# ZhengyiLuo/SMPLSim

Hardware: AMD Instinct MI355X
Metric: env-steps/sec (whole node), 4096-env SMPL rollout at 1/2/4/8 MI355X (higher is better)
Workload: dtype f32

## Files before the change

smplsim_amd/csrc/ss_api.h:

```cpp
#pragma once
#include <cassert>
#include <cstdlib>
#include <new>
#include <string>

#include "ss_imfused.h"
#include "ss_mjcf.h"
#include "ss_tables.h"

namespace ss {
inline std::string &last_error() { static thread_local std::string e; return e; }
inline std::string *&error_slot() { static thread_local std::string *p = nullptr; return p; }
struct HandleScope {
  template <class H> explicit HandleScope(const H *handle) { error_slot() = handle ? &handle->err : nullptr; }
  ~HandleScope() { error_slot() = nullptr; }
};
}

struct ss_model {
  ss::HostModel hm;
  int device = 0;
  uint32_t *d_shared = nullptr;
  ss::real *d_bodyc = nullptr, *d_candc = nullptr;
  int32_t *d_candb = nullptr;
// ... 28 lines not shown
  const float *fall_actions = nullptr;
  void *d_im = nullptr;
  ss_imitation_io im_io{};
};

template <class BE>
struct ss_api {
  static int fail(int code, const std::string &msg) {
    ss::last_error() = msg;
    if (ss::error_slot()) *ss::error_slot() = msg;
    return code;
  }

  static int model_create(const ss_model_desc *d, int device, ss_model **out) {
    if (!d || !out) return fail(SS_ERR_INVALID, "null argument");
    return model_create_shapes(d, 1, device, out);
  }
  template <class T> static bool up(T *&dst, const std::vector<T> &v) {
    const size_t bytes = v.size() * sizeof(T);
    dst = static_cast<T *>(BE::alloc(bytes ? bytes : 4));
    if (dst && bytes && !BE::upload(dst, v.data(), bytes)) { BE::free_(dst); dst = nullptr; }
    return dst != nullptr;
  }
  static int model_create_shapes(const ss_model_desc *d, int num_shapes, int device, ss_model **out) {
    if (!d || !out || num_shapes < 1) return fail(SS_ERR_INVALID, "null argument or num_shapes < 1");
    ss_model *m = new (std::nothrow) ss_model();
    if (!m) return fail(SS_ERR_NOMEM, "out of host memory");
    ss::HostModel &hm = m->hm;
    const std::string refusal = ss::build_host_model(d, num_shapes, getenv("SS_NO_ALIAS_LAYOUT") != nullptr, hm);
    if (!refusal.empty()) { delete m; return fail(SS_ERR_INVALID, refusal); }
    if (num_shapes > 1 && 12 * hm.h_sc.nb > hm.h_sc.l_Wst - hm.h_sc.l_IA) { delete m; return fail(SS_ERR_LDS, "no room for the per-env body offsets"); }
    m->num_shapes = num_shapes; m->device = device;
    if (!BE::set_device(device)) { delete m; return fail(SS_ERR_HIP, "cannot select device"); }
    if (!(up(m->d_shared, hm.shared) && up(m->d_bodyc, hm.bodyc) && up(m->d_candc, hm.candc) && up(m->d_candb, hm.candb) && up(m->d_pairs, hm.pairs) && up(m->d_geomc, hm.geomc))) {
      model_destroy(m);
      return fail(SS_ERR_HIP, "device table upload failed");
    }
    *out = m;
    return SS_OK;
  }
  static void model_destroy(ss_model *m) {
    if (!m) return;
    BE::free_(m->d_shared); BE::free_(m->d_bodyc); BE::free_(m->d_candc); BE::free_(m->d_candb); BE::free_(m->d_pairs); BE::free_(m->d_geomc);
    delete m;
  }
  static int batch_create(const ss_model *m, const ss_env_cfg *cfg, const ss_state *st, ss_batch **out) {
    if (!m || !cfg || !st || !out) return fail(SS_ERR_INVALID, "null argument");
    if (st->num_envs < 1) return fail(SS_ERR_INVALID, "num_envs must be positive");
    if (!st->qpos || !st->qvel || !st->qpos_prev || !st->qvel_prev || !st->qacc_warm || !st->body_vel || !st->touch ||
        !st->cur_t || !st->task || !st->nwarn || !st->solver_iters)
      return fail(SS_ERR_INVALID, "every ss_state buffer must be provided");
    if (cfg->control_mode < SS_CTRL_UHC_PD || cfg->control_mode > SS_CTRL_DEFAULT) return fail(SS_ERR_INVALID, "unknown control_mode");
    if (cfg->control_mode == SS_CTRL_SIMPLE_PID && (!st->pid_integral || !st->pid_last_error || !st->pid_started))
      return fail(SS_ERR_INVALID, "control_mode simple_pid needs the pid_* state buffers");
    if (cfg->self_obs_v != 1 && cfg->self_obs_v != 2) return fail(SS_ERR_INVALID, "self_obs_v must be 1 or 2");
    if (cfg->control_freq_inv < 1) return fail(SS_ERR_INVALID, "control_freq_inv must be >= 1");
    if (m->num_shapes > 1 && !st->shape_id) return fail(SS_ERR_INVALID, "a model with several shapes needs ss_state.shape_id");
    if (m->num_shapes == 1 && st->shape_id) return fail(SS_ERR_INVALID, "ss_state.shape_id given for a single-shape model");
    if (cfg->self_collision && !m->d_pairs) return fail(SS_ERR_INVALID, "model has no pair table");
    if (cfg->self_collision && !m->hm.self_collision_unavailable.empty()) return fail(SS_ERR_INVALID, m->hm.self_collision_unavailable.c_str());
    if (cfg->task == SS_TASK_REACH && (cfg->reach_body < 0 || cfg->reach_body >= m->hm.h.nb)) return fail(SS_ERR_INVALID, "reach_body out of range");
    const ss::Hdr &h = m->hm.h;
    if (ss::kernel_variant(h) < 0) return fail(SS_ERR_INVALID, "model too large for the compiled kernel variants");
    ss_batch *b = new (std::nothrow) ss_batch();
    if (!b) return fail(SS_ERR_NOMEM, "out of host memory");
    b->m = m; b->cfg = *cfg; b->st = *st;
    if (b->cfg.newton_iters <= 0) b->cfg.newton_iters = 100;
    b->cfg.solver_tolerance = (float)((cfg->solver_tolerance > 0.f ? (double)cfg->solver_tolerance : 1e-8) * m->hm.meaninertia * (h.nv > 1 ? h.nv : 1));
    b->obs_size = ss::obs_size(h, *cfg);
    size_t shared_b = (size_t)((h.shared_words + 3) & ~3) * 4;
    const size_t env_b = (size_t)(cfg->self_collision ? m->hm.sc.env_floats : h.env_floats) * sizeof(ss::real);
    int cap = BE::lds_capacity();
    const size_t pool_b = cfg->self_collision ? (size_t)ss::ss_pool_floats(m->hm.sc) * sizeof(ss::real) : 0;
    int e = (int)((cap - (long)shared_b - (long)pool_b) / (long)env_b);
    if (e < 1) { batch_destroy(b); return fail(SS_ERR_LDS, "model does not fit in LDS"); }
    { const int mw = BE::max_waves(ss::kernel_variant(h), cfg->self_collision); if (e > mw) e = mw; }
    { const char *cap = getenv("SS_ENVS_PER_WG"); if (cap && atoi(cap) > 0 && atoi(cap) < e) e = atoi(cap); }
    b->envs_per_wg = e;
    b->lds_bytes = shared_b + (size_t)e * env_b + pool_b;
#ifdef SS_PROFILE
    b->d_prof = (unsigned long long *)BE::alloc(64 * sizeof(unsigned long long));
    if (b->d_prof) { unsigned long long z[64] = {0}; BE::upload(b->d_prof, z, sizeof z); }
#endif
    if (!BE::set_device(m->device)) { batch_destroy(b); return fail(SS_ERR_HIP, "cannot select device"); }
    b->d_counter = (int32_t *)BE::alloc(2 * sizeof(int32_t));
    const int32_t zeros[2] = {0, 0};
    if (!b->d_counter || !BE::upload(b->d_counter, zeros, sizeof zeros)) { batch_destroy(b); return fail(SS_ERR_NOMEM, "device allocation failed"); }
    *out = b;
    return SS_OK;
  }
  static ss::KArgs base_args(const ss_batch *b, int mode) {
    ss::KArgs k{};
    const ss_model *m = b->m;
    k.h = b->cfg.self_collision ? m->hm.h_sc : m->hm.h; k.cfg = b->cfg; k.st = b->st;
    k.shared_g = m->d_shared; k.bodyc = m->d_bodyc; k.candc = m->d_candc; k.candb = m->d_candb;
    k.illegal_mask = m->hm.illegal_mask;
    k.hc = m->hm.hc;
    k.sc = m->hm.sc; k.pairs = m->d_pairs; k.geomc = m->d_geomc; k.dbg_self = ss_batch::R(b->dbg_self);
    k.mode = mode; k.nsub = b->cfg.control_freq_inv; k.obs_size = b->obs_size;
    k.work_counter = b->d_counter + b->parity; k.work_counter_next = b->d_counter + (b->parity ^ 1);
    k.obs_stride = b->obs_size;
    k.prof = b->d_prof;
    k.order = b->order;
// ... 248 lines not shown
```

smplsim_amd/csrc/ss_env_kernel.h:

```cpp
#pragma once
#include <hip/hip_runtime.h>

#include "ss_api.h"
#include "ss_kernel.h"
#include "ss_wave_gpu.h"

#ifndef SS_MAX_THREADS
#define SS_MAX_THREADS 768
#endif
#ifndef SS_MAX_THREADS_X
#define SS_MAX_THREADS_X 448
#endif
#ifndef SS_MAX_THREADS_SC
#define SS_MAX_THREADS_SC 512
#endif

namespace ss {
typedef void (*kern_t)(const KArgs);
kern_t pick_kernel_selfcol(const KernelKey &key, const Hdr &h, const HdrC &hc);
kern_t pick_kernel_imitation(const KernelKey &key, const Hdr &h, const HdrC &hc);
kern_t pick_kernel_imitation_selfcol(const KernelKey &key, const Hdr &h, const HdrC &hc);
kern_t pick_kernel_x(const KernelKey &key, const Hdr &h, const HdrC &hc);
}

namespace {

template <int DOFP, int CANDP, int SLOTP, int NPASS, int MAXT, bool BODYOUT, bool SHAPED, class HT = ss::HdrRuntime, bool SELFCOL = false, bool IMIT = false, bool CFORCE = false>
__global__ void __launch_bounds__(MAXT) ss_env_kernel(const ss::KArgs k) {
  extern __shared__ __align__(16) uint32_t lds[];
  if (blockIdx.x == 0 && threadIdx.x == 0) *k.work_counter_next = 0;
  for (int i = threadIdx.x; i < k.h.shared_words; i += blockDim.x) lds[i] = k.shared_g[i];
  if constexpr (SELFCOL)
    if (threadIdx.x == 0 && ss::ss_pool_floats(k.sc) > 0)
      *reinterpret_cast<int *>(reinterpret_cast<float *>(lds + ((k.h.shared_words + 3) & ~3)) + (size_t)(blockDim.x >> 6) * k.sc.env_floats) = 0;
  __syncthreads();
  const int wave = __builtin_amdgcn_readfirstlane(threadIdx.x >> 6);
  const int slice = SELFCOL ? k.sc.env_floats : HT::view(k.h).env_floats;
  float *L = reinterpret_cast<float *>(lds + ((k.h.shared_words + 3) & ~3)) + (size_t)wave * slice;
  float *pool = nullptr;
  if constexpr (SELFCOL) {
    if (ss::ss_pool_floats(k.sc) > 0) {
      pool = reinterpret_cast<float *>(lds + ((k.h.shared_words + 3) & ~3)) + (size_t)(blockDim.x >> 6) * slice;
    }
  }
  WaveGpu w{(int)(threadIdx.x & 63)};
  const int total_waves = (int)(gridDim.x * (blockDim.x >> 6));
  bool first = true;
  for (;;) {
    int env = wave * (int)gridDim.x + (int)blockIdx.x;
    if (!first) {
      if (w.ln == 0) env = atomicAdd(k.work_counter, 1) + total_waves;
      env = __builtin_amdgcn_readfirstlane(env);
    }
    first = false;
    if (env >= k.st.num_envs) break;
    if (k.order) env = __builtin_amdgcn_readfirstlane(k.order[env]);
    int mode = k.mode;
    if constexpr (IMIT) {
      const ss::mo::ImFused *f = static_cast<const ss::mo::ImFused *>(k.im);
      ss::run_env<WaveGpu, DOFP, CANDP, SLOTP, NPASS, BODYOUT, SHAPED, HT, SELFCOL, IMIT, CFORCE>(&w, &k, lds, L, env, mode, pool);
      w.sync();
      if (ss::mo::fused_after_step(&w, f, k.im_rand, env)) {
        ss::run_env<WaveGpu, DOFP, CANDP, SLOTP, NPASS, BODYOUT, SHAPED, HT, SELFCOL, IMIT, CFORCE>(&w, &k, lds, L, env, ss::MODE_RESET, pool);
        w.sync();
        ss::mo::fused_after_reset(&w, f, env);
      }
      continue;
    }
    for (int rep = 0; rep < 2; rep++) {
      const bool again = ss::run_env<WaveGpu, DOFP, CANDP, SLOTP, NPASS, BODYOUT, SHAPED, HT, SELFCOL, IMIT, CFORCE>(&w, &k, lds, L, env, mode, pool);
      w.sync();
      if (!again) break;
      mode = ss::MODE_RESET;
    }
  }
// ... 8 lines not shown
```

smplsim_amd/csrc/ss_hdr.h:

```cpp
#pragma once
#include <stdint.h>

#include "../../include/smplsim_hip.h"

#ifdef SS_F64
namespace ss { typedef double real; }
#define SS_M(fn) fn
#define SS_LS_TOL_EFF 1e-13
#define SS_ROUND_REL 2.2e-15
#define SS_DG_NOISE 1.8e-15
#define SS_LS_MAXIT 60
#else
namespace ss { typedef float real; }
#define SS_M(fn) fn##f
#define SS_LS_TOL_EFF SS_LS_TOL
#define SS_ROUND_REL 2e-6f
#define SS_DG_NOISE 1e-6f
#define SS_LS_MAXIT 16
#endif

namespace ss {

constexpr int kWave = 64;
constexpr int kBodyC = 16;
constexpr int kDofC = 12;
constexpr int kCandC = 8;

struct Hdr {
  int nb, nn, nv, nq, nu, ncand, nlev, a_stride, nbox, nslot, maxlev;
  int l_Rloc, l_w2;
  unsigned long long arm_lean;
  int o_dofc, o_boff, o_chainnode, o_ndepth, l_act, o_bparent, o_sumsmall, o_sumbig, o_sumcover, n_sumsmall, n_sumbig, shared_words;
  int l_q, l_v, l_a, l_tau, l_Fb, l_Pb, l_delta, l_diag, l_S, l_Ab, l_An, l_Aown, l_IA, l_Ubuf, l_Wst,
      l_R, l_r, l_Gb, l_tmp, l_V, l_Iown, ia_stride, env_floats;
  real dt, grav, margin, mu, solimp[5], K, B;
  real qpos0_root[3];
};

struct Layout {
  int l_q, l_v, l_a, l_tau, l_Fb, l_Pb, l_delta, l_diag, l_S, l_Ab, l_An, l_Aown, l_IA, l_Ubuf, l_Wst, l_R, l_r, l_Gb, l_tmp, l_V, l_Iown,
      ia_stride, l_act, env_floats, a_stride, l_Rloc, l_w2;
};
constexpr Layout make_layout(int nb, int maxlev, bool alias_w = false) {
  const int nn = nb + 1, nv = 6 + 3 * (nb - 1);
  Layout y{};
  int o = 0;
  auto take = [&](int n) { int r = o; o += (n + 3) & ~3; return r; };
  y.l_q = take(nv + 1); y.l_v = take(nv); y.l_a = take(nv); y.l_tau = take(nv);
  y.l_Fb = take(6 * nb);
  y.l_act = alias_w ? o : take(nv - 6);
  y.l_delta = take(nv);
// ... 17 lines not shown
    y.l_Wst = y.l_Aown;
    y.l_R = o - 12 * nb; y.l_r = y.l_R + 9 * nb;
    (void)gb; (void)t6;
    y.env_floats = o;
    return y;
  }
  y.a_stride = 21;
  y.l_Aown = take(21 * nb);
  y.ia_stride = 0;
  const int gb = (6 * nb + 3) & ~3;
  const int ia_need = 48 * maxlev > gb + 6 * nn ? 48 * maxlev : gb + 6 * nn;
  y.l_IA = take(ia_need);
  y.l_Gb = y.l_IA; y.l_tmp = y.l_IA + gb;
  y.l_Ubuf = 24 * maxlev <= 8 * nn ? y.l_An : take(24 * maxlev);
  y.l_Wst = take(24 * nn);
  y.l_R = y.l_Wst; y.l_r = y.l_Wst + 9 * nb;
  y.l_Rloc = y.l_IA; y.l_w2 = y.l_Wst + 12 * nb;
  y.env_floats = o;
  return y;
}
inline void apply_layout(Hdr &g, const Layout &y) {
  g.l_q = y.l_q; g.l_v = y.l_v; g.l_a = y.l_a; g.l_tau = y.l_tau; g.l_Fb = y.l_Fb; g.l_act = y.l_act; g.l_delta = y.l_delta; g.l_Pb = y.l_Pb; g.l_V = y.l_V;
  g.l_diag = y.l_diag; g.l_S = y.l_S; g.l_Ab = y.l_Ab; g.l_Iown = y.l_Iown; g.l_An = y.l_An; g.l_Aown = y.l_Aown; g.ia_stride = y.ia_stride;
  g.l_IA = y.l_IA; g.l_Gb = y.l_Gb; g.l_tmp = y.l_tmp; g.l_Ubuf = y.l_Ubuf; g.l_Wst = y.l_Wst; g.l_R = y.l_R; g.l_r = y.l_r;
  g.a_stride = y.a_stride; g.l_Rloc = y.l_Rloc; g.l_w2 = y.l_w2;
  g.env_floats = y.env_floats;
}
constexpr bool alias_layout_fits(int nb, int maxlev, int nslot) {
  const int nn = nb + 1;
  const Layout y = make_layout(nb, maxlev, true);
  return ((6 * nb + 3) & ~3) <= 48 * maxlev && y.l_w2 + ((6 * nn + 3) & ~3) <= y.l_R && 13 * nslot <= y.l_R - y.l_An;
}

constexpr int kMaxSelf = SS_MAX_SELF_CONTACTS;
constexpr int kSelfRec = 24;
constexpr int kSelfCand = 64;
constexpr int kCandRec = 8;
constexpr int kGeomC = 16;
constexpr int kDenseMaxRows = 64;
struct HdrSC {
  int npair;
  int l_H, l_g, l_list, l_Wst2, hloc, o_sctab, l_gc, l_tab, nmax, l_cand, l_zb;
  int env_floats;
};
constexpr int kDenseTile = 16;
constexpr int dense_tile_rows(int nblock) { return (3 * nblock + 1 + kDenseTile - 1) / kDenseTile; }
constexpr int dense_floats(int np) {
  const int t = (np - 1) / kDenseTile;
  return kDenseTile * kDenseTile * (t * (t + 1) / 2) + kDenseTile * (t + 1) * (np - kDenseTile * t);
}
constexpr int kDenseExtra = 256;
constexpr HdrSC make_layout_sc(int nb, int base_floats, int l_An) {
  HdrSC y{};
  int o = base_floats;
  auto take = [&](int n) { int r = o; o += (n + 3) & ~3; return r; };
  y.nmax = nb + 1 < kDenseMaxRows ? nb + 1 : kDenseMaxRows;
  y.l_H = l_An;
  take(kDenseExtra);
  y.hloc = o - y.l_H;
  y.l_g = take(kDenseTile * dense_tile_rows(y.nmax)); y.l_list = take(64);
  const int w2 = 24 * (nb + 1) > kCandRec * kSelfCand ? 24 * (nb + 1) : kCandRec * kSelfCand;
  y.l_Wst2 = take(w2); y.l_cand = y.l_Wst2;
  y.l_gc = take(3 * nb); y.l_zb = take(3 * nb); y.l_tab = take(3 * nb);
  y.env_floats = o;
  return y;
}
constexpr int ss_pool_floats(const HdrSC &y) { return dense_floats(3 * y.nmax + 1) > y.hloc ? 4 + ((dense_floats(3 * y.nmax + 1) + 3) & ~3) : 0; }

struct HdrC {
  int nlev;
  int o_lev;
  int root;
  int pel_level;
  unsigned long long nkpack[2];
  unsigned long long cpack;
  unsigned long long chain;
  unsigned long long neg;
};

#if defined(__HIPCC__)
#define SS_HD __host__ __device__ inline __attribute__((always_inline))
#else
#define SS_HD inline __attribute__((always_inline))
#endif
SS_HD int hdr_o_arm(const Hdr &h) { return (int)(h.arm_lean & 0xffffffffull); }
SS_HD bool hdr_lean(const Hdr &h) { return (h.arm_lean >> 32) != 0ull; }
struct HdrRuntime {
  typedef const Hdr &type;
  static constexpr bool fixed = false;
  static SS_HD bool lean(const Hdr &h) { return hdr_lean(h); }
  static constexpr bool maybe_lean = true;
  static SS_HD type view(const Hdr &h) { return h; }
  typedef const HdrC &tree_type;
  static SS_HD tree_type tree(const HdrC &c) { return c; }
};
template <int NLEV, int ROOT, int PEL, unsigned long long NK0, unsigned long long CP, unsigned long long CH, unsigned long long NG>
struct TreeFixed {
  static constexpr int nlev = NLEV, root = ROOT, pel_level = PEL;
  static constexpr unsigned long long nkpack[2] = {NK0, 0ull};
  static constexpr unsigned long long cpack = CP, chain = CH, neg = NG;
  int o_lev;
};
template <int NB, int MAXLEV, bool ALIAS = false>
struct HdrFixed {
  static constexpr Layout LY = make_layout(NB, MAXLEV, ALIAS);
  static constexpr int nb = NB, nn = NB + 1, nv = 6 + 3 * (NB - 1), nq = 7 + 3 * (NB - 1), maxlev = MAXLEV;
  static constexpr int l_q = LY.l_q, l_v = LY.l_v, l_a = LY.l_a, l_tau = LY.l_tau, l_Fb = LY.l_Fb, l_Pb = LY.l_Pb, l_delta = LY.l_delta,
                       l_diag = LY.l_diag, l_S = LY.l_S, l_Ab = LY.l_Ab, l_An = LY.l_An, l_Aown = LY.l_Aown, l_IA = LY.l_IA,
                       l_Ubuf = LY.l_Ubuf, l_Wst = LY.l_Wst, l_R = LY.l_R, l_r = LY.l_r, l_Gb = LY.l_Gb, l_tmp = LY.l_tmp, l_V = LY.l_V,
                       l_Iown = LY.l_Iown, ia_stride = LY.ia_stride, l_act = LY.l_act, env_floats = LY.env_floats,
                       a_stride = LY.a_stride, l_Rloc = LY.l_Rloc, l_w2 = LY.l_w2;
  const int &nu, &ncand, &nlev, &nbox, &nslot;
  const int &o_dofc, &o_boff, &o_chainnode, &o_ndepth, &o_bparent, &o_sumsmall, &o_sumbig, &o_sumcover, &n_sumsmall, &n_sumbig,
      &shared_words;
  const real &dt, &grav, &margin, &mu;
  const real (&solimp)[5];
  const real &K, &B;
  const real (&qpos0_root)[3];
  SS_HD explicit HdrFixed(const Hdr &h)
      : nu(h.nu), ncand(h.ncand), nlev(h.nlev), nbox(h.nbox), nslot(h.nslot), o_dofc(h.o_dofc),
        o_boff(h.o_boff), o_chainnode(h.o_chainnode), o_ndepth(h.o_ndepth), o_bparent(h.o_bparent),
        o_sumsmall(h.o_sumsmall), o_sumbig(h.o_sumbig), o_sumcover(h.o_sumcover), n_sumsmall(h.n_sumsmall), n_sumbig(h.n_sumbig),
        shared_words(h.shared_words), dt(h.dt), grav(h.grav), margin(h.margin), mu(h.mu), solimp(h.solimp), K(h.K), B(h.B),
        qpos0_root(h.qpos0_root) {}
};
template <int NB, int MAXLEV, int NLEV, int ROOT, int PEL, unsigned long long NK0, unsigned long long CP, unsigned long long CH, unsigned long long NG, bool ALIAS = false, bool LEAN = ALIAS>
struct HdrFixedT {
  typedef const HdrFixed<NB, MAXLEV, ALIAS> type;
  static constexpr bool fixed = true;
  static SS_HD constexpr bool lean(const Hdr &) { return LEAN; }
  static constexpr bool maybe_lean = LEAN;
  static SS_HD HdrFixed<NB, MAXLEV, ALIAS> view(const Hdr &h) { return HdrFixed<NB, MAXLEV, ALIAS>(h); }
  typedef const TreeFixed<NLEV, ROOT, PEL, NK0, CP, CH, NG> tree_type;
  static SS_HD TreeFixed<NLEV, ROOT, PEL, NK0, CP, CH, NG> tree(const HdrC &c) { TreeFixed<NLEV, ROOT, PEL, NK0, CP, CH, NG> t; t.o_lev = c.o_lev; return t; }
  static bool matches(const Hdr &h, const HdrC &c) {
    return h.nb == NB && h.maxlev == MAXLEV && h.a_stride == (ALIAS ? 24 : 21) && hdr_lean(h) == LEAN && h.env_floats == HdrFixed<NB, MAXLEV, ALIAS>::env_floats && c.nlev == NLEV && c.root == ROOT && c.pel_level == PEL && c.nkpack[0] == NK0 && c.nkpack[1] == 0ull && c.cpack == CP && c.chain == CH && c.neg == NG;
  }
};


typedef HdrFixedT<24, 5, 6, 10, 2, 0x333431ull, 0x1253ull, 0x1cull, 0x3ull> HdrSmplFixed;
typedef HdrFixedT<52, 12, 7, 11, 3, 0xbbb3233ull, 0x9a89ull, 0x33ull, 0x7ull, true> HdrSmplxFixed;
typedef HdrFixedT<52, 12, 7, 11, 3, 0xbbb3233ull, 0x9a89ull, 0x33ull, 0x7ull, false, true> HdrSmplxFixedSC;

inline int kernel_variant(const Hdr &h) {
  const int dofp = (h.nv + 63) / 64, candp = (h.ncand + 63) / 64, slotp = (h.nslot + 63) / 64, npass = (h.maxlev + 7) / 8;
  if (dofp <= 2 && candp <= 2 && slotp <= 1 && npass <= 1) return 0;
  if (dofp <= 3 && candp <= 3 && slotp <= 2 && npass <= 2) return 1;
  return -1;
}

template <class H> constexpr int shape_stride(const H &h) { return h.nb * kBodyC + ((h.nv + 3) & ~3); }

enum { MODE_STEP = 0, MODE_SUBSTEP = 1, MODE_RESET = 2, MODE_KINEMATICS = 3, MODE_DEBUG_FORWARD = 4 };

struct KArgs {
  Hdr h;
  ss_env_cfg cfg;
  ss_state st;
  const uint32_t *shared_g;
  const real *bodyc;
  const real *candc;
  const int32_t *candb;
  uint64_t illegal_mask;
  int mode, nsub, obs_size;
  const real *actions;
  const real *task_rand;
  const real *fall_actions;
  const uint8_t *mask;
  unsigned long long *prof;
  const int32_t *order;
  int32_t *work_counter;
  real *obs, *reward;
  int fused_reset;
  real *obs2;
  const real *task_rand2;
  uint8_t *terminated, *truncated;
  real *out0, *out1, *out2;
  HdrSC sc;
  const int32_t *pairs;
  const real *geomc;
  real *dbg_self;
  int obs_stride;
  const void *im;
  const float *im_rand;
  int32_t *work_counter_next;
  real *power;
  int32_t *self_trunc;
  HdrC hc;
  real *cforce;
};

inline int env_slice_floats(const KArgs &k) { return k.cfg.self_collision ? k.sc.env_floats : k.h.env_floats; }
inline size_t launch_lds_bytes(const KArgs &k, int e) {
  return (size_t)((k.h.shared_words + 3) & ~3) * 4 + ((size_t)e * env_slice_floats(k) + (k.cfg.self_collision ? ss_pool_floats(k.sc) : 0)) * sizeof(real);
}

struct KernelKey { int variant; bool bodyout, shaped, selfcol, imit, cforce; };
inline KernelKey kernel_key(const KArgs &k) {
  KernelKey key{kernel_variant(k.h), false, k.st.shape_id != nullptr, k.cfg.self_collision != 0, k.im != nullptr, false};
  const bool wanted = (k.out0 || k.power || k.cforce) && (k.mode == MODE_STEP || k.mode == MODE_RESET);
  key.bodyout = wanted || key.shaped || key.selfcol || key.imit;
  key.cforce = k.cforce && k.mode == MODE_STEP;
  return key;
}

struct LaunchGeometry { int wgs, envs_per_wg; size_t lds_bytes; };
inline LaunchGeometry launch_geometry(int nenv, int cus, int envs_per_wg, int fixed_epw, int max_wgs, size_t lds_capacity, size_t lds_fixed, size_t lds_per_env) {
  const int per_cu = (nenv + cus - 1) / cus;
  if (fixed_epw > 0) envs_per_wg = fixed_epw;
  else if (per_cu < envs_per_wg) envs_per_wg = per_cu < 1 ? 1 : per_cu;
  LaunchGeometry g{(nenv + envs_per_wg - 1) / envs_per_wg, envs_per_wg, lds_fixed + (size_t)envs_per_wg * lds_per_env};
  const int resident = cus * (int)(lds_capacity / g.lds_bytes > 0 ? lds_capacity / g.lds_bytes : 1);
  if (g.wgs > resident) g.wgs = resident;
  if (max_wgs > 0 && g.wgs > max_wgs) g.wgs = max_wgs;
  return g;
}

}
```

smplsim_amd/csrc/ss_kernel.h:

```cpp
#pragma once
#include <math.h>
#include <stdint.h>
#include <stdlib.h>
#include <stdio.h>

#include "ss_hdr.h"
#include "ss_selfcol.h"

#if defined(__HIPCC__)
#define SS_DEV __device__ __forceinline__
#else
#define SS_DEV inline
#endif

#ifdef SS_PROFILE
#define SS_T0() unsigned long long t__ = w->clock()
#define SS_TICK(id) do { unsigned long long n__ = w->clock(); sim.prof[id] += n__ - t__; t__ = n__; } while (0)
#else
#define SS_T0() do {} while (0)
#define SS_TICK(id) do {} while (0)
#endif

#ifndef SS_LS_TOL
#define SS_LS_TOL 1e-2f
// ... 191 lines not shown
#pragma unroll
      for (int u = 1; u < 8; u++) part[u] = u < n ? part[u] : 0.f;
      out[b * NC + c] = ((part[0] + part[1]) + (part[2] + part[3])) + ((part[4] + part[5]) + (part[6] + part[7]));
    }
    if (h.n_sumbig == 0) return;
    w->sync();
    for (int idx = lane; idx < NC * h.n_sumbig; idx += 64) {
      const int o = idx / NC, c = idx - o * NC, e = ti(h.o_sumbig, o), b = e & 255, start = (e >> 8) & 4095, cnt = e >> 20;
      real acc = 0.f;
      for (int j = 0; j < cnt; j += 4) {
        real part[4];
#pragma unroll
        for (int u = 0; u < 4; u++) {
          const int t = ti(h.o_sumcover, start + (j + u < cnt ? j + u : j));
          part[u] = (t < 64 ? in : out)[(t & 63) * NC + c];
        }
#pragma unroll
        for (int u = 1; u < 4; u++) part[u] = j + u < cnt ? part[u] : 0.f;
        acc += (part[0] + part[1]) + (part[2] + part[3]);
      }
      out[b * NC + c] = acc;
    }
  }

  SS_DEV void body_accel(const real *x, real *A, real *tmp) {
    typename HT::type h = HT::view(k->h);
    for (int idx = lane; idx < 6 * h.nn; idx += 64) {
      int n = idx / 6, c = idx - 6 * n, d = 3 * n;
      tmp[idx] = S[6 * d + c] * x[d] + S[6 * d + 6 + c] * x[d + 1] + S[6 * d + 12 + c] * x[d + 2];
    }
    w->sync();
    chain_sum(tmp, A);
  }
  SS_DEV void chain_sum(const real *tmp, real *A, const real *tmp2 = nullptr, real *A2 = nullptr) {
    typename HT::type h = HT::view(k->h);
    for (int idx = lane; idx < 6 * h.nb; idx += 64) {
      int b = idx / 6, c = idx - 6 * b, n = b + 1;
      const int dn = ti(h.o_ndepth, n), row = h.o_chainnode + n * h.nlev;
      real s = 0.f, s2 = 0.f;
      for (int kk = 0; kk <= dn; kk += 4) {
        const int k1 = kk + 1 <= dn ? kk + 1 : kk, k2 = kk + 2 <= dn ? kk + 2 : kk, k3 = kk + 3 <= dn ? kk + 3 : kk;
        const int n0 = ti(row, kk), n1 = ti(row, k1), n2 = ti(row, k2), n3 = ti(row, k3);
        const real a0 = tmp[6 * n0 + c], a1 = tmp[6 * n1 + c], a2 = tmp[6 * n2 + c], a3 = tmp[6 * n3 + c];
        s += (a0 + (kk + 1 <= dn ? a1 : 0.f)) + ((kk + 2 <= dn ? a2 : 0.f) + (kk + 3 <= dn ? a3 : 0.f));
        if (tmp2) {
          const real e0 = tmp2[6 * n0 + c], e1 = tmp2[6 * n1 + c], e2 = tmp2[6 * n2 + c], e3 = tmp2[6 * n3 + c];
          s2 += (e0 + (kk + 1 <= dn ? e1 : 0.f)) + ((kk + 2 <= dn ? e2 : 0.f) + (kk + 3 <= dn ? e3 : 0.f));
        }
      }
      A[idx] = s;
      if (tmp2) A2[idx] = s2;
    }
  }


  SS_DEV void forward_kin(bool with_dyn, bool write_sensors) {
    fresh();
    typename HT::type h = HT::view(k->h);
    SS_FT0();
    real vb[6] = {0, 0, 0, 0, 0, 0}, ab[6] = {0, 0, 0, 0, 0, 0};
    real Rb[9] = {1, 0, 0, 0, 1, 0, 0, 0, 1}, rb[3] = {0, 0, 0};
    real bc[kBodyC];
    {
      const float4_t *src = reinterpret_cast<const float4_t *>(bodyc() + (lane < h.nb ? lane : 0) * kBodyC);
      const float4_t b0 = src[0], b1 = src[1], b2 = src[2], b3 = src[3];
      bc[0] = b0.x; bc[1] = b0.y; bc[2] = b0.z; bc[3] = b0.w; bc[4] = b1.x; bc[5] = b1.y; bc[6] = b1.z; bc[7] = b1.w;
      bc[8] = b2.x; bc[9] = b2.y; bc[10] = b2.z; bc[11] = b2.w; bc[12] = b3.x; bc[13] = b3.y; bc[14] = b3.z; bc[15] = b3.w;
    }
// ... 2208 lines not shown
```

smplsim_amd/csrc/ss_tables.h:

```cpp
#pragma once
#include <algorithm>
#include <cmath>
#include <cstdint>
#include <cstring>
#include <string>
#include <vector>

#include "../../include/smplsim_hip.h"
#include "ss_hdr.h"

namespace ss {

struct HostModel {
  Hdr h{}, h_sc{};
  HdrC hc{};
  HdrSC sc{};
  uint64_t illegal_mask = 0;
  double meaninertia = 0;
  std::string self_collision_unavailable;
  std::vector<uint32_t> shared;
  std::vector<int32_t> candb;
  std::vector<real> bodyc, candc, geomc;
  std::vector<int32_t> pairs;
};
struct Tree {
  std::vector<int> parent, chainnode, ndepth; int nlev = 0;
  std::vector<int> sum_small, sum_big, sum_cover;
  HdrC hc{}; int maxlev = 1;
  std::vector<int> levrec, towards, joint, negated;
};
struct Topology {
  Hdr h{};
  Tree tree;
  std::vector<real> dofc;
  std::vector<int32_t> candb, pair_ids;
  uint64_t illegal_mask = 0;
};
struct Shape {
  std::vector<real> bodyc, invw, boff, candc, geomc;
  std::vector<int32_t> reach;
  double meaninertia = 0;
};

inline void quat2mat(const double *q, double *m) {
  double w = q[0], x = q[1], y = q[2], z = q[3];
  double n = std::sqrt(w * w + x * x + y * y + z * z);
  w /= n; x /= n; y /= n; z /= n;
  m[0] = 1 - 2 * (y * y + z * z); m[1] = 2 * (x * y - w * z); m[2] = 2 * (x * z + w * y);
  m[3] = 2 * (x * y + w * z); m[4] = 1 - 2 * (x * x + z * z); m[5] = 2 * (y * z - w * x);
  m[6] = 2 * (x * z - w * y); m[7] = 2 * (y * z + w * x); m[8] = 1 - 2 * (x * x + y * y);
}
inline void body_frame_inertia(const ss_model_desc &d, int b, double *I) {
  double R[9]; quat2mat(d.body_iquat + 4 * b, R);
  for (int i = 0; i < 3; i++) for (int j = 0; j < 3; j++) {
    double s = 0; for (int k = 0; k < 3; k++) s += R[3 * i + k] * d.body_inertia[3 * b + k] * R[3 * j + k];
    I[3 * i + j] = s;
  }
}

// ... 26 lines not shown
inline const char *validate(const ss_model_desc &d) {
  const int nb = d.nbody, nv = 6 + 3 * (nb - 1);
  if (nb < 1 || nb > 63) return "nbody must be in [1,63]";
  if (d.body_parent[0] != -1) return "body 0 must be the root";
  for (int b = 1; b < nb; b++) if (d.body_parent[b] < 0 || d.body_parent[b] >= b) return "parents must precede children";
  for (int b = 2; b < nb; b++) {
    int a = b - 1;
    while (a > 0 && a != d.body_parent[b]) a = d.body_parent[a];
    if (a != d.body_parent[b]) return "bodies must be in depth-first order";
  }
  for (int i = 0; i < 6; i++) if (d.dof_armature[i] != 0.0) return "armature on the free joint is not supported";
  std::vector<bool> driven(nv, false);
  for (int i = 0; i < d.nu; i++) {
    const int dof = d.actuator_dof[i];
    if (dof < 6 || dof >= nv || driven[dof]) return "bad actuator_dof";
    driven[dof] = true;
  }
  for (int b = 0; b < nb; b++) if (d.geom_type[b] != SS_GEOM_BOX && d.geom_type[b] != SS_GEOM_CAPSULE && d.geom_type[b] != SS_GEOM_SPHERE) return "unknown geom type";
  if (d.impratio != 1.0) return "impratio != 1 is not supported";
  return nullptr;
}

inline const char *node_tree(Tree &t) {
  const int nb = (int)t.parent.size(), nn = nb + 1;
  std::vector<int> nparent(nn); t.ndepth.assign(nn, 0);
  nparent[0] = -1; nparent[1] = 0; t.ndepth[1] = 1;
  for (int b = 1; b < nb; b++) { nparent[b + 1] = t.parent[b] + 1; t.ndepth[b + 1] = t.ndepth[t.parent[b] + 1] + 1; }
  t.nlev = 1 + *std::max_element(t.ndepth.begin(), t.ndepth.end());
  if (t.nlev > 32) return "tree too deep";
  t.chainnode.assign(nn * t.nlev, 0);
  for (int n = 0; n < nn; n++)
    for (int a = n; a >= 0; a = nparent[a]) t.chainnode[n * t.nlev + t.ndepth[a]] = a;
  return nullptr;
}

inline void subtree_sum_tables(Tree &t) {
  const int nb = (int)t.parent.size(), kSmall = 8;
  std::vector<int> subsize(nb, 1), order(nb);
  for (int b = nb - 1; b >= 1; b--) subsize[t.parent[b]] += subsize[b];
  for (int b = 0; b < nb; b++) order[b] = b;
  std::stable_sort(order.begin(), order.end(), [&](int x, int y) { return subsize[x] > subsize[y]; });
  std::vector<std::vector<int>> cov(nb);
  for (int b = nb - 1; b >= 0; b--) {
    if (subsize[b] <= kSmall) continue;
    cov[b].push_back(b);
    for (int c = b + 1; c < nb; c++) {
      if (t.parent[c] != b) continue;
      if (subsize[c] <= kSmall) cov[b].push_back(64 + c);
      else cov[b].insert(cov[b].end(), cov[c].begin(), cov[c].end());
    }
  }
  for (int b : order) {
    if (subsize[b] <= kSmall) { t.sum_small.push_back(b | (subsize[b] << 8)); continue; }
    t.sum_big.push_back(b | ((int)t.sum_cover.size() << 8) | ((int)cov[b].size() << 20));
    t.sum_cover.insert(t.sum_cover.end(), cov[b].begin(), cov[b].end());
  }
}

inline int centre_of_tree(const Tree &t, std::vector<int> &dep, std::vector<int> &tw) {
  const int nb = (int)t.parent.size();
  std::vector<std::vector<int>> adj(nb);
  for (int b = 1; b < nb; b++) { adj[b].push_back(t.parent[b]); adj[t.parent[b]].push_back(b); }
  auto bfs = [&](int c) {
    dep.assign(nb, -1); tw.assign(nb, -1);
    std::vector<int> q{c}; dep[c] = 0;
    for (size_t i = 0; i < q.size(); i++) for (int o : adj[q[i]]) if (dep[o] < 0) { dep[o] = dep[q[i]] + 1; tw[o] = q[i]; q.push_back(o); }
// ... 162 lines not shown
    t.pair_ids.push_back(first | ((first == i ? j : i) << 8));
    const float rs = (float)((reach(i) + reach(j) + d.margin) * (1.0 + 1e-5));
    int32_t bits; std::memcpy(&bits, &rs, 4);
    s.reach.push_back(bits);
  }
  s.geomc.assign((size_t)nb * kGeomC, real(0));
  for (int b = 0; b < nb; b++) {
    real *c = &s.geomc[(size_t)b * kGeomC];
    double G[9]; quat2mat(d.geom_quat + 4 * b, G);
    for (int k = 0; k < 3; k++) { c[k] = (real)d.geom_pos[3 * b + k]; c[3 + k] = (real)d.geom_size[3 * b + k]; }
    if (d.geom_type[b] == SS_GEOM_SPHERE) { c[4] = 0; c[5] = 0; }
    for (int k = 0; k < 9; k++) c[6 + k] = (real)G[k];
    c[15] = (real)d.geom_type[b];
  }
}

inline void physics_scalars(const ss_model_desc &d, Hdr &h) {
  h.dt = (real)d.timestep; h.grav = (real)d.gravity; h.margin = (real)d.margin; h.mu = (real)d.friction;
  for (int k = 0; k < 5; k++) h.solimp[k] = (real)d.solimp[k];
  const double dmax = d.solimp[1], tc = d.solref[0] < 2 * d.timestep ? 2 * d.timestep : d.solref[0];
  h.K = (real)(1.0 / (dmax * dmax * tc * tc * d.solref[1] * d.solref[1]));
  h.B = (real)(2.0 / (dmax * tc));
  for (int k = 0; k < 3; k++) h.qpos0_root[k] = (real)d.qpos0[k];
}

inline const char *describe(const ss_model_desc &d, const Topology *like, Topology &t, Shape &s) {
  if (const char *e = validate(d)) return e;
  const int nb = d.nbody;
  Hdr &h = t.h;
  h.nb = nb; h.nn = nb + 1; h.nv = 6 + 3 * (nb - 1); h.nq = h.nv + 1; h.nu = d.nu;
  t.tree.parent.assign(d.body_parent, d.body_parent + nb);
  if (!like || like->tree.parent != t.tree.parent) {
    if (const char *e = node_tree(t.tree)) return e;
    subtree_sum_tables(t.tree);
    if (const char *e = elimination_tree(t.tree)) return e;
  }
  t.dofc = dof_constants(d);
  if (const char *e = body_constants(d, s)) return e;
  floor_candidates(d, t, s);
  pair_and_geom_tables(d, t, s);
  physics_scalars(d, h);
  return nullptr;
}

inline bool same_topology(const Topology &a, const Topology &b) {
  const Hdr &h = a.h, &g = b.h;
  return h.nb == g.nb && h.nu == g.nu && h.ncand == g.ncand && h.nbox == g.nbox && h.nslot == g.nslot && a.tree.parent == b.tree.parent &&
         a.dofc.size() == b.dofc.size() && !std::memcmp(a.dofc.data(), b.dofc.data(), a.dofc.size() * sizeof(real)) && a.candb == b.candb &&
         a.pair_ids == b.pair_ids && a.illegal_mask == b.illegal_mask && h.dt == g.dt && h.grav == g.grav && h.margin == g.margin && h.mu == g.mu &&
         h.K == g.K && h.B == g.B;
}

inline std::vector<uint32_t> assemble_blob(const Topology &t, const Shape *shape, bool lean, Hdr &h, HdrC &hc) {
  std::vector<uint32_t> S;
  auto push_i = [&](const std::vector<int> &v) { int o = (int)S.size(); S.insert(S.end(), v.begin(), v.end()); return o; };
  const Tree &tr = t.tree;
  h.o_chainnode = push_i(tr.chainnode); h.o_ndepth = push_i(tr.ndepth); h.o_bparent = push_i(tr.parent);
  h.o_sumsmall = push_i(tr.sum_small); h.o_sumbig = push_i(tr.sum_big); h.o_sumcover = push_i(tr.sum_cover);
  hc.o_lev = push_i(tr.levrec);
  while (S.size() % 4) S.push_back(0u);
  const int o_real = (int)S.size(), real0 = o_real / (int)(sizeof(real) / 4);
  std::vector<real> dofc = t.dofc, boff(3 * h.nb, real(0)), F;
  if (shape) { boff = shape->boff; for (int i = 0; i < h.nv; i++) dofc[i * kDofC + 4] = shape->invw[i]; }
  auto push_r = [&](const std::vector<real> &v) { int o = real0 + (int)F.size(); F.insert(F.end(), v.begin(), v.end()); return o; };
  int o_arm = 0;
  if (lean) {
// ... 24 lines not shown
  if (13 * m.h.nslot > plain.l_Wst - plain.l_An) return "contact record buffer does not fit";
  m.h_sc = m.h; apply_layout(m.h_sc, plain);
  apply_layout(m.h, alias ? make_layout(m.h.nb, m.h.maxlev, true) : plain);
  m.sc = make_layout_sc(m.h.nb, plain.env_floats, plain.l_An);
  return nullptr;
}

inline void body_contact_tables(const Topology &top, HostModel &m) {
  const Tree &t = top.tree; const int nb = m.h.nb;
  m.sc.npair = (int)top.pair_ids.size(); m.sc.o_sctab = (int)m.pairs.size();
  for (int b = 0; b < nb; b++) {
    unsigned long long pm = 0ull;
    for (int a = b; a != t.hc.root; a = t.towards[a]) pm |= 1ull << a;
    m.pairs.push_back(t.towards[b] | (t.joint[b] << 8) | (t.negated[b] << 16));
    m.pairs.push_back((int32_t)(uint32_t)(pm & 0xFFFFFFFFull)); m.pairs.push_back((int32_t)(uint32_t)(pm >> 32));
  }
  if (nb < 2) m.self_collision_unavailable = "a single body has no body-body contacts";
  else if (8 * t.hc.nlev > 64) m.self_collision_unavailable = "elimination tree deeper than 8 levels (one lane per (joint, row) of a contact's joints)";
  else if (12 * 2 * t.hc.nlev > m.sc.l_tab - m.sc.l_gc) m.self_collision_unavailable = "tree too deep for its body count (body-body contacts need 4 x levels <= bodies)";
}

inline std::string build_host_model(const ss_model_desc *d, int num_shapes, bool plain_layout, HostModel &out) {
  Topology top; Shape first;
  for (int s = 0; s < num_shapes; s++) {
    Topology t; Shape sh;
    if (const char *e = describe(d[s], s ? &top : nullptr, t, sh)) return num_shapes > 1 ? "shape " + std::to_string(s) + ": " + e : std::string(e);
    if (s && !same_topology(t, top)) return "shape " + std::to_string(s) + " differs from shape 0 in more than its geometry";
    append_shape(t, sh, num_shapes > 1, out);
    if (s == 0) { top = std::move(t); first = std::move(sh); }
  }
  const Tree &tree = top.tree;
  Hdr &h = out.h = top.h;
  h.nlev = tree.nlev; h.maxlev = tree.maxlev; h.n_sumsmall = (int)tree.sum_small.size(); h.n_sumbig = (int)tree.sum_big.size();
  out.hc = tree.hc; out.candb = top.candb; out.illegal_mask = top.illegal_mask; out.meaninertia = first.meaninertia;
  const bool alias = h.nb > 32 && alias_layout_fits(h.nb, h.maxlev, h.nslot) && !plain_layout;
  out.shared = assemble_blob(top, num_shapes == 1 ? &first : nullptr, alias, h, out.hc);
  if (const char *e = lds_layouts(alias, out)) return e;
  body_contact_tables(top, out);
  return "";
}

inline int obs_size(const Hdr &h, const ss_env_cfg &c) {
  int nd = 3 * (h.nb - 1);
  int n = (c.root_height_obs ? 1 : 0) + nd + (c.self_obs_v == 1 ? 6 * h.nb + 6 + nd : 12 * h.nb);
  if (c.task == SS_TASK_SPEED || c.task == SS_TASK_REACH) n += 3;
  if (c.task == SS_TASK_GETUP) n += 1;
  return n;
}

}
```

Baseline: 2.821 million.

## Pack per-node ancestor chains into aligned LDS records for vectorized chain sums

Builds per-node records holding depth and ancestor node indices as bytes, padded to 16-byte units. These are appended after the shared tables in global memory and copied into LDS. For fixed-header kernels, chain_sum now reads each record with 128-bit LDS loads and sums a fixed, unrolled number of levels with predication. This replaces the per-level table lookups in a variable-length loop, trading extra LDS table space (possibly fewer envs per workgroup) for fewer dependent LDS reads and less branching.

```diff
diff --git a/smplsim_amd/csrc/ss_api.h b/smplsim_amd/csrc/ss_api.h
--- a/smplsim_amd/csrc/ss_api.h
+++ b/smplsim_amd/csrc/ss_api.h
@@ -84,7 +84,10 @@
     if (num_shapes > 1 && 12 * hm.h_sc.nb > hm.h_sc.l_Wst - hm.h_sc.l_IA) { delete m; return fail(SS_ERR_LDS, "no room for the per-env body offsets"); }
     m->num_shapes = num_shapes; m->device = device;
     if (!BE::set_device(device)) { delete m; return fail(SS_ERR_HIP, "cannot select device"); }
-    if (!(up(m->d_shared, hm.shared) && up(m->d_bodyc, hm.bodyc) && up(m->d_candc, hm.candc) && up(m->d_candb, hm.candb) && up(m->d_pairs, hm.pairs) && up(m->d_geomc, hm.geomc))) {
+    std::vector<uint32_t> tables = hm.shared;
+    tables.resize((size_t)ss::chain_rec_goffset(hm.h), 0u);
+    tables.insert(tables.end(), hm.chainrec.begin(), hm.chainrec.end());
+    if (!(up(m->d_shared, tables) && up(m->d_bodyc, hm.bodyc) && up(m->d_candc, hm.candc) && up(m->d_candb, hm.candb) && up(m->d_pairs, hm.pairs) && up(m->d_geomc, hm.geomc))) {
       model_destroy(m);
       return fail(SS_ERR_HIP, "device table upload failed");
     }
@@ -120,7 +123,7 @@
     if (b->cfg.newton_iters <= 0) b->cfg.newton_iters = 100;
     b->cfg.solver_tolerance = (float)((cfg->solver_tolerance > 0.f ? (double)cfg->solver_tolerance : 1e-8) * m->hm.meaninertia * (h.nv > 1 ? h.nv : 1));
     b->obs_size = ss::obs_size(h, *cfg);
-    size_t shared_b = (size_t)((h.shared_words + 3) & ~3) * 4;
+    size_t shared_b = (size_t)ss::lds_table_words(h) * 4;
     const size_t env_b = (size_t)(cfg->self_collision ? m->hm.sc.env_floats : h.env_floats) * sizeof(ss::real);
     int cap = BE::lds_capacity();
     const size_t pool_b = cfg->self_collision ? (size_t)ss::ss_pool_floats(m->hm.sc) * sizeof(ss::real) : 0;
diff --git a/smplsim_amd/csrc/ss_env_kernel.h b/smplsim_amd/csrc/ss_env_kernel.h
--- a/smplsim_amd/csrc/ss_env_kernel.h
+++ b/smplsim_amd/csrc/ss_env_kernel.h
@@ -29,18 +29,19 @@
 __global__ void __launch_bounds__(MAXT) ss_env_kernel(const ss::KArgs k) {
   extern __shared__ __align__(16) uint32_t lds[];
   if (blockIdx.x == 0 && threadIdx.x == 0) *k.work_counter_next = 0;
-  for (int i = threadIdx.x; i < k.h.shared_words; i += blockDim.x) lds[i] = k.shared_g[i];
+  const int tables = ss::lds_table_words(k.h), rec_shift = ss::chain_rec_goffset(k.h) - ss::chain_rec_offset(k.h);
+  for (int i = threadIdx.x; i < tables; i += blockDim.x) lds[i] = k.shared_g[i < k.h.shared_words ? i : i + rec_shift];
   if constexpr (SELFCOL)
     if (threadIdx.x == 0 && ss::ss_pool_floats(k.sc) > 0)
-      *reinterpret_cast<int *>(reinterpret_cast<float *>(lds + ((k.h.shared_words + 3) & ~3)) + (size_t)(blockDim.x >> 6) * k.sc.env_floats) = 0;
+      *reinterpret_cast<int *>(reinterpret_cast<float *>(lds + tables) + (size_t)(blockDim.x >> 6) * k.sc.env_floats) = 0;
   __syncthreads();
   const int wave = __builtin_amdgcn_readfirstlane(threadIdx.x >> 6);
   const int slice = SELFCOL ? k.sc.env_floats : HT::view(k.h).env_floats;
-  float *L = reinterpret_cast<float *>(lds + ((k.h.shared_words + 3) & ~3)) + (size_t)wave * slice;
+  float *L = reinterpret_cast<float *>(lds + tables) + (size_t)wave * slice;
   float *pool = nullptr;
   if constexpr (SELFCOL) {
     if (ss::ss_pool_floats(k.sc) > 0) {
-      pool = reinterpret_cast<float *>(lds + ((k.h.shared_words + 3) & ~3)) + (size_t)(blockDim.x >> 6) * slice;
+      pool = reinterpret_cast<float *>(lds + tables) + (size_t)(blockDim.x >> 6) * slice;
     }
   }
   WaveGpu w{(int)(threadIdx.x & 63)};
diff --git a/smplsim_amd/csrc/ss_hdr.h b/smplsim_amd/csrc/ss_hdr.h
--- a/smplsim_amd/csrc/ss_hdr.h
+++ b/smplsim_amd/csrc/ss_hdr.h
@@ -17,6 +17,12 @@
 #define SS_ROUND_REL 2e-6f
 #define SS_DG_NOISE 1e-6f
 #define SS_LS_MAXIT 16
+#endif
+
+#if defined(__HIPCC__)
+#define SS_HD __host__ __device__ inline __attribute__((always_inline))
+#else
+#define SS_HD inline __attribute__((always_inline))
 #endif
 
 namespace ss {
@@ -100,6 +106,10 @@
   return ((6 * nb + 3) & ~3) <= 48 * maxlev && y.l_w2 + ((6 * nn + 3) & ~3) <= y.l_R && 13 * nslot <= y.l_R - y.l_An;
 }
 
+constexpr int chain_rec_bytes(int nlev) { return (1 + nlev + 15) & ~15; }
+constexpr int chain_rec_words(int nn, int nlev) { return nn * (chain_rec_bytes(nlev) / 4); }
+constexpr int fixed_chain_levels(int nb) { return nb == 24 ? 10 : nb == 52 ? 12 : 0; }
+
 constexpr int kMaxSelf = SS_MAX_SELF_CONTACTS;
 constexpr int kSelfRec = 24;
 constexpr int kSelfCand = 64;
@@ -146,13 +156,11 @@
   unsigned long long neg;
 };
 
-#if defined(__HIPCC__)
-#define SS_HD __host__ __device__ inline __attribute__((always_inline))
-#else
-#define SS_HD inline __attribute__((always_inline))
-#endif
 SS_HD int hdr_o_arm(const Hdr &h) { return (int)(h.arm_lean & 0xffffffffull); }
 SS_HD bool hdr_lean(const Hdr &h) { return (h.arm_lean >> 32) != 0ull; }
+SS_HD int chain_rec_offset(const Hdr &h) { return (h.shared_words + 3) & ~3; }
+SS_HD int chain_rec_goffset(const Hdr &h) { return hdr_lean(h) ? ((h.o_dofc + h.nv * kDofC) * (int)(sizeof(real) / 4) + 3) & ~3 : chain_rec_offset(h); }
+SS_HD int lds_table_words(const Hdr &h) { return (chain_rec_offset(h) + chain_rec_words(h.nn, h.nlev)) & ~3; }
 struct HdrRuntime {
   typedef const Hdr &type;
   static constexpr bool fixed = false;
@@ -173,6 +181,7 @@
 struct HdrFixed {
   static constexpr Layout LY = make_layout(NB, MAXLEV, ALIAS);
   static constexpr int nb = NB, nn = NB + 1, nv = 6 + 3 * (NB - 1), nq = 7 + 3 * (NB - 1), maxlev = MAXLEV;
+  static constexpr int chain_levels = fixed_chain_levels(NB);
   static constexpr int l_q = LY.l_q, l_v = LY.l_v, l_a = LY.l_a, l_tau = LY.l_tau, l_Fb = LY.l_Fb, l_Pb = LY.l_Pb, l_delta = LY.l_delta,
                        l_diag = LY.l_diag, l_S = LY.l_S, l_Ab = LY.l_Ab, l_An = LY.l_An, l_Aown = LY.l_Aown, l_IA = LY.l_IA,
                        l_Ubuf = LY.l_Ubuf, l_Wst = LY.l_Wst, l_R = LY.l_R, l_r = LY.l_r, l_Gb = LY.l_Gb, l_tmp = LY.l_tmp, l_V = LY.l_V,
@@ -202,7 +211,7 @@
   typedef const TreeFixed<NLEV, ROOT, PEL, NK0, CP, CH, NG> tree_type;
   static SS_HD TreeFixed<NLEV, ROOT, PEL, NK0, CP, CH, NG> tree(const HdrC &c) { TreeFixed<NLEV, ROOT, PEL, NK0, CP, CH, NG> t; t.o_lev = c.o_lev; return t; }
   static bool matches(const Hdr &h, const HdrC &c) {
-    return h.nb == NB && h.maxlev == MAXLEV && h.a_stride == (ALIAS ? 24 : 21) && hdr_lean(h) == LEAN && h.env_floats == HdrFixed<NB, MAXLEV, ALIAS>::env_floats && c.nlev == NLEV && c.root == ROOT && c.pel_level == PEL && c.nkpack[0] == NK0 && c.nkpack[1] == 0ull && c.cpack == CP && c.chain == CH && c.neg == NG;
+    return h.nb == NB && h.nlev == fixed_chain_levels(NB) && h.maxlev == MAXLEV && h.a_stride == (ALIAS ? 24 : 21) && hdr_lean(h) == LEAN && h.env_floats == HdrFixed<NB, MAXLEV, ALIAS>::env_floats && c.nlev == NLEV && c.root == ROOT && c.pel_level == PEL && c.nkpack[0] == NK0 && c.nkpack[1] == 0ull && c.cpack == CP && c.chain == CH && c.neg == NG;
   }
 };
 
@@ -261,7 +270,7 @@
 
 inline int env_slice_floats(const KArgs &k) { return k.cfg.self_collision ? k.sc.env_floats : k.h.env_floats; }
 inline size_t launch_lds_bytes(const KArgs &k, int e) {
-  return (size_t)((k.h.shared_words + 3) & ~3) * 4 + ((size_t)e * env_slice_floats(k) + (k.cfg.self_collision ? ss_pool_floats(k.sc) : 0)) * sizeof(real);
+  return (size_t)lds_table_words(k.h) * 4 + ((size_t)e * env_slice_floats(k) + (k.cfg.self_collision ? ss_pool_floats(k.sc) : 0)) * sizeof(real);
 }
 
 struct KernelKey { int variant; bool bodyout, shaped, selfcol, imit, cforce; };
diff --git a/smplsim_amd/csrc/ss_kernel.h b/smplsim_amd/csrc/ss_kernel.h
--- a/smplsim_amd/csrc/ss_kernel.h
+++ b/smplsim_amd/csrc/ss_kernel.h
@@ -247,8 +247,60 @@
     w->sync();
     chain_sum(tmp, A);
   }
+  static constexpr bool kChainRec = HT::fixed;
+  static constexpr int chain_levels_c() { if constexpr (HT::fixed) return HT::type::chain_levels; else return 1; }
+  static constexpr int kRecUnits = chain_rec_bytes(chain_levels_c()) / 16;
+  struct alignas(16) rec4_t { uint32_t x, y, z, w; };
+  SS_DEV const uint32_t *chain_recs() const {
+#if defined(__HIP_DEVICE_COMPILE__)
+    return T + chain_rec_offset(k->h);
+#else
+    return T + chain_rec_goffset(k->h);
+#endif
+  }
+  SS_DEV void rec_read(int n, uint32_t *rw) const {
+    const rec4_t *p = reinterpret_cast<const rec4_t *>(chain_recs()) + n * kRecUnits;
+#pragma unroll
+    for (int u = 0; u < kRecUnits; u++) { const rec4_t v = p[u]; rw[4 * u] = v.x; rw[4 * u + 1] = v.y; rw[4 * u + 2] = v.z; rw[4 * u + 3] = v.w; }
+  }
+  SS_DEV static int rec_depth(const uint32_t *rw) { return (int)(rw[0] & 0xffu); }
+  SS_DEV static int rec_node(const uint32_t *rw, int lev) { return (int)((rw[(1 + lev) >> 2] >> (8 * ((1 + lev) & 3))) & 0xffu); }
+  template <bool TWO>
+  SS_DEV void chain_sum_rec(const real *tmp, real *A, const real *tmp2, real *A2) {
+    typename HT::type h = HT::view(k->h);
+    constexpr int NL = chain_levels_c(), NG = (NL + 3) / 4;
+#pragma unroll 1
+    for (int idx = lane; idx < 6 * h.nb; idx += 64) {
+      const int b = idx / 6, c = idx - 6 * b;
+      uint32_t rw[4 * kRecUnits];
+      rec_read(b + 1, rw);
+      const int dn = rec_depth(rw);
+      const real *p = tmp + c, *p2 = tmp2 + c;
+      real a[4 * NG], e[4 * NG];
+#pragma unroll
+      for (int u = 0; u < 4 * NG; u++) {
+        const int nu = 6 * rec_node(rw, u < NL ? u : NL - 1);
+        a[u] = p[nu];
+        if constexpr (TWO) e[u] = p2[nu];
+      }
+      real s = 0.f, s2 = 0.f;
+#pragma unroll
+      for (int g = 0; g < NG; g++) {
+        const int kk = 4 * g;
+        const real ga = (a[kk] + (kk + 1 <= dn ? a[kk + 1] : 0.f)) + ((kk + 2 <= dn ? a[kk + 2] : 0.f) + (kk + 3 <= dn ? a[kk + 3] : 0.f));
+        s = kk <= dn ? s + ga : s;
+        if constexpr (TWO) {
+          const real ge = (e[kk] + (kk + 1 <= dn ? e[kk + 1] : 0.f)) + ((kk + 2 <= dn ? e[kk + 2] : 0.f) + (kk + 3 <= dn ? e[kk + 3] : 0.f));
+          s2 = kk <= dn ? s2 + ge : s2;
+        }
+      }
+      A[idx] = s;
+      if constexpr (TWO) A2[idx] = s2;
+    }
+  }
   SS_DEV void chain_sum(const real *tmp, real *A, const real *tmp2 = nullptr, real *A2 = nullptr) {
     typename HT::type h = HT::view(k->h);
+    if constexpr (kChainRec) { if (tmp2) chain_sum_rec<true>(tmp, A, tmp2, A2); else chain_sum_rec<false>(tmp, A, tmp, A); return; }
     for (int idx = lane; idx < 6 * h.nb; idx += 64) {
       int b = idx / 6, c = idx - 6 * b, n = b + 1;
       const int dn = ti(h.o_ndepth, n), row = h.o_chainnode + n * h.nlev;
diff --git a/smplsim_amd/csrc/ss_tables.h b/smplsim_amd/csrc/ss_tables.h
--- a/smplsim_amd/csrc/ss_tables.h
+++ b/smplsim_amd/csrc/ss_tables.h
@@ -19,12 +19,14 @@
   double meaninertia = 0;
   std::string self_collision_unavailable;
   std::vector<uint32_t> shared;
+  std::vector<uint32_t> chainrec;
   std::vector<int32_t> candb;
   std::vector<real> bodyc, candc, geomc;
   std::vector<int32_t> pairs;
 };
 struct Tree {
   std::vector<int> parent, chainnode, ndepth; int nlev = 0;
+  std::vector<uint32_t> chainrec;
   std::vector<int> sum_small, sum_big, sum_cover;
   HdrC hc{}; int maxlev = 1;
   std::vector<int> levrec, towards, joint, negated;
@@ -117,6 +119,16 @@
   for (int n = 0; n < nn; n++)
     for (int a = n; a >= 0; a = nparent[a]) t.chainnode[n * t.nlev + t.ndepth[a]] = a;
   return nullptr;
+}
+
+inline void chain_records(Tree &t) {
+  const int nn = (int)t.ndepth.size(), nby = chain_rec_bytes(t.nlev);
+  t.chainrec.assign((size_t)chain_rec_words(nn, t.nlev), 0u);
+  auto put = [&](int n, int i, uint32_t v) { t.chainrec[(size_t)n * (nby / 4) + i / 4] |= v << (8 * (i & 3)); };
+  for (int n = 0; n < nn; n++) {
+    put(n, 0, (uint32_t)t.ndepth[n]);
+    for (int k = 0; k + 1 < nby; k++) put(n, 1 + k, (uint32_t)(k <= t.ndepth[n] ? t.chainnode[n * t.nlev + k] : n));
+  }
 }
 
 inline void subtree_sum_tables(Tree &t) {
@@ -345,6 +357,7 @@
   t.tree.parent.assign(d.body_parent, d.body_parent + nb);
   if (!like || like->tree.parent != t.tree.parent) {
     if (const char *e = node_tree(t.tree)) return e;
+    chain_records(t.tree);
     subtree_sum_tables(t.tree);
     if (const char *e = elimination_tree(t.tree)) return e;
   }
@@ -435,7 +448,7 @@
   const Tree &tree = top.tree;
   Hdr &h = out.h = top.h;
   h.nlev = tree.nlev; h.maxlev = tree.maxlev; h.n_sumsmall = (int)tree.sum_small.size(); h.n_sumbig = (int)tree.sum_big.size();
-  out.hc = tree.hc; out.candb = top.candb; out.illegal_mask = top.illegal_mask; out.meaninertia = first.meaninertia;
+  out.hc = tree.hc; out.chainrec = tree.chainrec; out.candb = top.candb; out.illegal_mask = top.illegal_mask; out.meaninertia = first.meaninertia;
   const bool alias = h.nb > 32 && alias_layout_fits(h.nb, h.maxlev, h.nslot) && !plain_layout;
   out.shared = assemble_blob(top, num_shapes == 1 ? &first : nullptr, alias, h, out.hc);
   if (const char *e = lds_layouts(alias, out)) return e;
```

Result: faster. 2.885 million (median of 6 runs) (+2.3%).
